# AutoGPTQ/AutoGPTQ

Hardware: AMD Instinct MI355X
Metric: int4 g128 QuantLinear fwd GB/s + tokens/s, Llama-7B shapes (higher is better)
Workload: dtype f16; 1 GPU; Llama-7B linear shapes (4096->4096 x4, 4096->11008 x2, 11008->4096) x 32 blocks = 224 layers, int4 g128 no act-order, M=1 rows per step, 128 launches/step in one hipGraph (q|k|v and gate|up of a block: one gptq_forward_multi launch each); layers=224, launches=128, parallelism=single

## Files before the change

autogptq_amd/csrc/gemv_shared.cuh:

```cuda
#pragma once
#include <type_traits>

#include "common.cuh"
#include "launch.h"

namespace gptq {

struct GemvParams {
    const unsigned* qweight;
    const unsigned* qzeros;
    const void* scales;
    const int* g_idx;
    const int* perm;
    const void* bias;
    const void* x;
    void* out;
    float* partial;
    int M, K, N, group_size, zero_mode;
    int units_total, units_per_split, chunk_units, ksplit;
    int gu_shift;
    int pair_off;
};
hipError_t launch_gemv_generic(const gptq_layer_t& L, const GemvPlan& pl, const GemvParams& p, hipStream_t st);

template <int CTRL> __device__ __forceinline__ float dpp_add(float v) {
    const int r = __builtin_amdgcn_update_dpp(0, __builtin_bit_cast(int, v), CTRL, 0xf, 0xf, false);
    return v + __builtin_bit_cast(float, r);
}
template <int LN> __device__ __forceinline__ float row_slot_sum(float v) {
    if constexpr (LN <= 4) v = dpp_add<0x124>(v);
    if constexpr (LN <= 8) v = dpp_add<0x128>(v);
    if constexpr (LN <= 16) v += __shfl_xor(v, 16, 64);
    if constexpr (LN <= 32) v += __shfl_xor(v, 32, 64);
    return v;
}

__device__ __forceinline__ float kslot_sum_swap(float v) {
    const unsigned u = __builtin_bit_cast(unsigned, v);
    const auto a = __builtin_amdgcn_permlane16_swap(u, u, false, false);
    const unsigned a0 = a[0], a1 = a[1];
    const unsigned s = as_u32(as_f32(a0) + as_f32(a1));
    const auto b = __builtin_amdgcn_permlane32_swap(s, s, false, false);
    const unsigned b0 = b[0], b1 = b[1];
    return as_f32(b0) + as_f32(b1);
}
template <int WN, int STRIDE> __device__ __forceinline__ float tree_sum(const float* r) {
    float a[WN];
#pragma unroll
    for (int w = 0; w < WN; ++w) a[w] = r[w * STRIDE];
#pragma unroll
    for (int off = 1; off < WN; off <<= 1)
#pragma unroll
        for (int i = 0; i < WN; i += 2 * off) a[i] += a[i + off];
    return a[0];
}
template <int WN, int STRIDE> __device__ __forceinline__ float seq_sum(const float* r) {
    float a[WN];
#pragma unroll
    for (int w = 0; w < WN; ++w) a[w] = r[w * STRIDE];
    float t = 0.f;
#pragma unroll
    for (int w = 0; w < WN; ++w) t += a[w];
    return t;
}

template <typename T> struct Mma4;
template <> struct Mma4<f16> {
    typedef _Float16 v4 __attribute__((ext_vector_type(4)));
    static __device__ __forceinline__ f32x4 run(u32x2 a, u32x2 b, f32x4 c) {
        return __builtin_amdgcn_mfma_f32_4x4x4f16(__builtin_bit_cast(v4, a), __builtin_bit_cast(v4, b), c, 0, 0, 0);
    }
    static __device__ __forceinline__ unsigned short bits_of_int(int d) { return as_u16((f16)(short)d); }
};
template <> struct Mma4<bf16> {
    typedef short v4 __attribute__((ext_vector_type(4)));
    static __device__ __forceinline__ f32x4 run(u32x2 a, u32x2 b, f32x4 c) {
        return __builtin_amdgcn_mfma_f32_4x4x4bf16_1k(__builtin_bit_cast(v4, a), __builtin_bit_cast(v4, b), c, 0, 0, 0);
    }
    static __device__ __forceinline__ unsigned short bits_of_int(int d) { return (unsigned short)(as_u32((float)d) >> 16); }
};

__device__ __forceinline__ void dma16_nt(const void* gsrc, unsigned lds_dst) {
    unsigned keep;
    asm volatile("s_mov_b32 %0, m0\n\ts_mov_b32 m0, %2\n\ts_nop 0\n\tglobal_load_lds_dwordx4 %1, off nt\n\ts_mov_b32 m0, %0"
                 : "=&s"(keep) : "v"(gsrc), "s"(lds_dst) : "memory");
}

template <bool NT> __device__ __forceinline__ void dma16_sv(__attribute__((address_space(1))) const char* sbase, unsigned voff, unsigned lds_dst) {
    if constexpr (NT) asm volatile("s_mov_b32 m0, %2\n\ts_nop 0\n\tglobal_load_lds_dwordx4 %0, %1 nt" : : "v"(voff), "s"(sbase), "s"(lds_dst) : "memory");
    else asm volatile("s_mov_b32 m0, %2\n\ts_nop 0\n\tglobal_load_lds_dwordx4 %0, %1" : : "v"(voff), "s"(sbase), "s"(lds_dst) : "memory");
}
template <int ROWS, bool NT>
__device__ __forceinline__ void stage_rows(__attribute__((address_space(1))) const char* const (&base)[ROWS], const unsigned (&lds)[ROWS], int tid, int w64, int step, int pieces) {
    if (w64 >= pieces) return;
    if (tid < pieces) {
#pragma unroll
        for (int r = 0; r < ROWS; ++r) dma16_sv<NT>(base[r], (unsigned)tid * 16u, lds[r] + (unsigned)w64 * 16u);
    }
    if (w64 + step >= pieces) return;
    if (tid + step < pieces) {
#pragma unroll
        for (int r = 0; r < ROWS; ++r) dma16_sv<NT>(base[r], (unsigned)(tid + step) * 16u, lds[r] + (unsigned)(w64 + step) * 16u);
    }
    if (__builtin_expect(w64 + 2 * step >= pieces, 1)) return;
    for (int a = 2 * step; w64 + a < pieces; a += step) {
        if (tid + a < pieces) {
#pragma unroll
            for (int r = 0; r < ROWS; ++r) dma16_sv<NT>(base[r], (unsigned)(tid + a) * 16u, lds[r] + (unsigned)(w64 + a) * 16u);
        }
    }
}
__device__ __forceinline__ int scalar_ge(int a, int b) {
    int r;
    asm("s_cmp_ge_i32 %1, %2\n\ts_cselect_b32 %0, 1, 0" : "=s"(r) : "s"(a), "s"(b) : "scc");
    return r;
}

struct GemvSeg {
    const unsigned* qweight;
    const unsigned* qzeros;
    const void* scales;
    const void* bias;
    void* out;
    int N;
    int blk_end;
    int col0;
    int pad_;
};
struct GemvStreamParams {
    GemvSeg seg[4];
    const void* x;
    unsigned long long* gran;
    unsigned* epochs;
    unsigned* err;
    int nseg, M, K, zero_mode, units_total, units_per_split, ksplit, gu_shift, nsum;
    unsigned max_spins;
};

template <int CT, int MT, typename T, typename PP = GemvStreamParams, typename SG = GemvSeg>
__device__ __forceinline__ void stream_finish(const PP& p, const SG& sg, int strip, int sidx, int ks, int N, const float* red, T* stage = nullptr) {
    const int tid = threadIdx.x, lane = tid & 63, wave = tid >> 6, W = blockDim.x >> 6;
    constexpr int E = MT * CT, ES = E + 4;
    unsigned tag = 0;
    if (p.ksplit > 1) {
        unsigned ep;
        asm volatile("s_load_dword %0, %1, 0x0\n\ts_waitcnt lgkmcnt(0)" : "=s"(ep) : "s"(p.epochs + sidx) : "memory");
        tag = 0x7FE00000u | ((ep + 1u) & 0x1FFFFFu);
    }
    const size_t slab = (size_t)p.M * p.nsum;
    bool gave_up = false;
    auto emit = [&](int e, float t) {
        const int m = e / CT, c = e % CT;
        const int n = strip * CT + c;
        if (n >= N || m >= p.M) return;
        if (p.ksplit > 1) {
            const size_t at = (size_t)m * p.nsum + sg.col0 + n;
            if (ks != 0) {
                const unsigned long long g8 = (unsigned long long)as_u32(t) | ((unsigned long long)tag << 32);
                __hip_atomic_store(p.gran + (size_t)(ks - 1) * slab + at, g8, __ATOMIC_RELAXED, __HIP_MEMORY_SCOPE_AGENT);
                return;
            }
            constexpr int KMAX = 8;
            unsigned long long v[KMAX - 1];
            unsigned pending = (1u << (p.ksplit - 1)) - 1u;
            for (unsigned spins = 0; pending; ++spins) {
#pragma unroll
                for (int k = 0; k < KMAX - 1; ++k)
                    if (pending & (1u << k)) v[k] = __hip_atomic_load(p.gran + (size_t)k * slab + at, __ATOMIC_RELAXED, __HIP_MEMORY_SCOPE_AGENT);
#pragma unroll
                for (int k = 0; k < KMAX - 1; ++k)
                    if ((pending & (1u << k)) && (unsigned)(v[k] >> 32) == tag) pending &= ~(1u << k);
                if (pending && spins > p.max_spins) { gave_up = true; break; }
                if (pending) __builtin_amdgcn_s_sleep(2);
            }
#pragma unroll
            for (int k = 0; k < KMAX - 1; ++k)
                if (k < p.ksplit - 1) t += as_f32((unsigned)(v[k] & 0xffffffffu));
#pragma unroll
            for (int k = 0; k < KMAX - 1; ++k)
                if (k < p.ksplit - 1) __hip_atomic_store(p.gran + (size_t)k * slab + at, 0ull, __ATOMIC_RELAXED, __HIP_MEMORY_SCOPE_AGENT);
        }
        if (sg.bias) t += DType<T>::to_f32(((const T*)sg.bias)[n]);
        const T o = DType<T>::from_f32(t);
        if (sg.out) ((T*)sg.out)[(size_t)m * N + n] = o;
        if (stage) stage[m * CT + c] = o;
    };
    if ((W & (W - 1)) == 0) {
        const int lw = __builtin_ctz((unsigned)W);
        const int w_of_lane = lane & (W - 1), e_of_lane = lane >> lw;
        for (int e0 = 0; e0 < E; e0 += 64) {
            const int e = e0 + wave * (64 >> lw) + e_of_lane;
            float t = (e < E) ? red[w_of_lane * ES + e] : 0.f;
            for (int off = 1; off < W; off <<= 1) t += __shfl_xor(t, off, 64);
            if (w_of_lane == 0 && e < E) emit(e, t);
        }
    } else {
        for (int e = tid; e < E; e += blockDim.x) {
            float t = 0.f;
            for (int w = 0; w < W; ++w) t += red[w * ES + e];
            emit(e, t);
        }
    }
    if (p.ksplit > 1 && ks == 0) {
        if (gave_up) __hip_atomic_store(p.err, 1u, __ATOMIC_RELAXED, __HIP_MEMORY_SCOPE_AGENT);
        __syncthreads();
        if (tid == 0) __hip_atomic_store(p.epochs + sidx, (tag & 0x1FFFFFu), __ATOMIC_RELAXED, __HIP_MEMORY_SCOPE_AGENT);
    }
}

template <int LN, int MT, typename T>
__device__ __forceinline__ void stream_epilogue(f32x4 (&acc)[MT], const GemvStreamParams& p, const GemvSeg& sg, int strip, int sidx, int ks, int N,
                                                float* red) {
    constexpr int CT = LN * 4;
    const int tid = threadIdx.x, lane = tid & 63, wave = tid >> 6, W = blockDim.x >> 6;
#pragma unroll
    for (int m = 0; m < MT; ++m)
#pragma unroll
        for (int c = 0; c < 4; ++c) acc[m][c] = row_slot_sum<LN>(acc[m][c]);
    constexpr int E = MT * CT, ES = E + 4;
    if (lane < LN) {
#pragma unroll
        for (int m = 0; m < MT; ++m) *(f32x4*)(red + wave * ES + m * CT + lane * 4) = acc[m];
    }
    __syncthreads();
    stream_finish<CT, MT, T>(p, sg, strip, sidx, ks, N, red);
}


}
```

autogptq_amd/csrc/gemv_tiled_kernel.cuh:

```cuda
#pragma once
#include <cstddef>

#include "gemv_shared.cuh"

namespace gptq {

struct TiledSeg {
    const void* bias;
    void* out;
    int N, col0;
};
struct PeerEpi {
    char* xbuf[2][GPTQ_PEER_MAX];
    unsigned* flags[GPTQ_PEER_MAX];
    unsigned* state;
    int world, rank;
    unsigned row_bytes, col_off_bytes, owners, pad_;
};
struct TiledParams {
    int blk_end[4];
    const void* x;
    int M, K;
    int chunks, chunks_per_split, ksplit, gu_shift, groups, xstride, waves;
    int pair_strips;
    const unsigned* tq[4];
    const void* cst[4];
    const int* perm[4];
    int xraw_off;
    int nseg, nsum;
    unsigned max_spins;
    TiledSeg seg[4];
    unsigned long long* gran;
    unsigned* epochs;
    unsigned* err;
    PeerEpi peer;
};
static_assert(offsetof(TiledParams, perm) == 128, "the entry batch of the decode-copy kernel is the first two cache lines of its arguments");

template <int BITS> struct TiledFmt;
template <> struct TiledFmt<4> { static constexpr int WPL = 4, KPL = 32, REC = 48, ZB = 1; };
template <> struct TiledFmt<8> { static constexpr int WPL = 4, KPL = 16, REC = 64, ZB = 2; };
template <> struct TiledFmt<3> { static constexpr int WPL = 3, KPL = 32, REC = 48, ZB = 1; };
template <> struct TiledFmt<2> { static constexpr int WPL = 2, KPL = 32, REC = 48, ZB = 1; };

#ifdef GPTQ_TILED_STAMPS
#define TILED_STAMP(i) (st_[i] = __builtin_amdgcn_s_memtime() | vz_)
#define TILED_STAMPS_OUT() stamps_out()
#define TILED_HOT_END() return
#else
#define TILED_HOT_END() __builtin_amdgcn_endpgm()
#define TILED_STAMP(i) ((void)0)
#define TILED_STAMPS_OUT() ((void)0)
#endif

template <int N_> struct WordsOf { typedef unsigned type __attribute__((ext_vector_type(N_))); };

template <int BITS, int MT, int U, typename T, int MAXW, int XM = 0, int ZM2 = 0>
__global__ void __launch_bounds__(MAXW * 64, MAXW == 16 ? 4 : 2) gemv_tiled_kernel(TiledParams p) {
#ifdef GPTQ_TILED_STAMPS
    unsigned long long st_[9] = {};
    unsigned vz_;
    asm volatile("v_mov_b32 %0, 0" : "=v"(vz_));
    st_[7] = __builtin_amdgcn_s_memrealtime() | vz_;
    TILED_STAMP(0);
    auto stamps_out = [&]() {
        st_[8] = __builtin_amdgcn_s_memrealtime() | vz_;
        unsigned long long* const dbg = p.gran;
        const int b = (int)blockIdx.x, nb = (int)gridDim.x;
        const int slot = b == 0 ? 0 : (b == 1 ? 1 : (b == nb / 2 ? 2 : (b == nb - 1 ? 3 : -1)));
        if (dbg != nullptr && p.ksplit == 1 && slot >= 0 && (threadIdx.x & 63) == 0) {
#pragma unroll
            for (int i = 0; i < 9; ++i) dbg[(slot * 16 + (int)(threadIdx.x >> 6)) * 16 + i] = st_[i];
        }
    };
#endif
    constexpr bool BF = std::is_same_v<T, bf16>;
    constexpr bool ACT = XM == 1, PEER = XM == 3;
    constexpr bool PAIR = XM == 4;
    constexpr bool MULTI = XM == 5 || XM == 6;
    constexpr int NSTR = PAIR ? 2 : (XM == 5 ? 4 : (XM == 6 ? 2 : 1));
    using F = TiledFmt<BITS>;
    constexpr int WPL = F::WPL, KPL = F::KPL, CKE = 4 * KPL, CHB = 64 * WPL * 4, REC = F::REC, NX = KPL / 8;
    constexpr int LKPL = KPL == 32 ? 5 : 4;
    typedef typename WordsOf<WPL>::type qvec;
    unsigned m_lo, m_hi, m_b, magic;
    asm("s_mov_b32 %0, 0x000f000f" : "=s"(m_lo));
    asm("s_mov_b32 %0, 0x00f000f0" : "=s"(m_hi));
    asm("s_mov_b32 %0, 0x00ff00ff" : "=s"(m_b));
    asm("v_mov_b32 %0, 0x64006400" : "=v"(magic));
    unsigned m2a, m2b, m2c, m2d, m2e;
    asm("s_mov_b32 %0, 0x00030003" : "=s"(m2a));
    asm("s_mov_b32 %0, 0x000c000c" : "=s"(m2b));
    asm("s_mov_b32 %0, 0x00300030" : "=s"(m2c));
    asm("s_mov_b32 %0, 0x00c000c0" : "=s"(m2d));
    asm("s_mov_b32 %0, 0x03000300" : "=s"(m2e));
    unsigned m3a, m3b, m3c;
    asm("s_mov_b32 %0, 0x00070007" : "=s"(m3a));
    asm("s_mov_b32 %0, 0x00380038" : "=s"(m3b));
    asm("s_mov_b32 %0, 0x01c001c0" : "=s"(m3c));
    extern __shared__ __attribute__((aligned(16))) char smem[];
    const int tid = threadIdx.x, lane = tid & 63;
    const int wave = __builtin_amdgcn_readfirstlane(tid >> 6);
    const int col = lane & 15, kb = lane >> 4;
    typedef unsigned u32x16 __attribute__((ext_vector_type(16)));
    typedef unsigned long long u64x8 __attribute__((ext_vector_type(8)));
    typedef unsigned long long u64x4 __attribute__((ext_vector_type(4)));
    static_assert(offsetof(TiledParams, x) == 16 && offsetof(TiledParams, M) == 24 && offsetof(TiledParams, chunks) == 32 && offsetof(TiledParams, pair_strips) == 60 &&
                  offsetof(TiledParams, tq) == 64 && offsetof(TiledParams, cst) == 96 && offsetof(TiledParams, perm) == 128 && offsetof(TiledParams, xraw_off) == 160, "the entry batch");
    u32x16 ha;
    u64x8 hb;
    [[maybe_unused]] u64x4 hp = {};
    [[maybe_unused]] int xraw_off = 0;
    {
        const auto kargs = __builtin_amdgcn_kernarg_segment_ptr();
        if constexpr (ACT)
            asm volatile("s_load_dwordx16 %0, %4, 0x0\n\ts_load_dwordx16 %1, %4, 0x40\n\ts_load_dwordx8 %2, %4, 0x80\n\ts_load_dword %3, %4, 0xa0\n\ts_waitcnt lgkmcnt(0)"
                         : "=&s"(ha), "=&s"(hb), "=&s"(hp), "=&s"(xraw_off) : "s"(kargs));
        else
            asm volatile("s_load_dwordx16 %0, %2, 0x0\n\ts_load_dwordx16 %1, %2, 0x40\n\ts_waitcnt lgkmcnt(0)" : "=&s"(ha), "=&s"(hb) : "s"(kargs));
    }
    const int be0 = (int)ha[0], be1 = (int)ha[1], be2 = (int)ha[2], Mrows = (int)ha[6], K = (int)ha[7], nchunks = (int)ha[8], cps = (int)ha[9], ksplit = (int)ha[10],
              gshift = (int)ha[11], G = (int)ha[12], xstride = (int)ha[13], W = (int)ha[14];
    [[maybe_unused]] const int hstrips = (int)ha[15];
    typedef __attribute__((address_space(1))) const char gchar;
    gchar* const xg = (gchar*)(((unsigned long long)ha[5] << 32) | ha[4]);
    int sidx = blockIdx.x, ks = 0, cb = 0, ce = nchunks, kbeg = 0, kend = K;
    if (__builtin_expect(ksplit != 1, 0)) {
        sidx = (int)blockIdx.x / ksplit; ks = (int)blockIdx.x - sidx * ksplit;
        cb = ks * cps; ce = min(cb + cps, nchunks);
        kbeg = cb * CKE; kend = min(ce * CKE, K);
    }
    unsigned long long tqs_ = hb[0], csts_ = hb[4];
    [[maybe_unused]] unsigned long long perm_ = hp[0];
    int sbase = 0, s = 0;
    if constexpr (ACT)
        asm("s_cmp_ge_i32 %[i], %[e0]\n\ts_cbranch_scc0 1f\n\t"
            "s_mov_b64 %[tq], %[tq1]\n\ts_mov_b64 %[cs], %[cs1]\n\ts_mov_b64 %[pm], %[pm1]\n\ts_mov_b32 %[sb], %[e0]\n\ts_mov_b32 %[s], 1\n\t"
            "s_cmp_ge_i32 %[i], %[e1]\n\ts_cselect_b64 %[tq], %[tq2], %[tq]\n\ts_cselect_b64 %[cs], %[cs2], %[cs]\n\ts_cselect_b64 %[pm], %[pm2], %[pm]\n\ts_cselect_b32 %[sb], %[e1], %[sb]\n\ts_cselect_b32 %[s], 2, %[s]\n\t"
            "s_cmp_ge_i32 %[i], %[e2]\n\ts_cselect_b64 %[tq], %[tq3], %[tq]\n\ts_cselect_b64 %[cs], %[cs3], %[cs]\n\ts_cselect_b64 %[pm], %[pm3], %[pm]\n\ts_cselect_b32 %[sb], %[e2], %[sb]\n\ts_cselect_b32 %[s], 3, %[s]\n"
            "1:"
            : [tq] "+&s"(tqs_), [cs] "+&s"(csts_), [pm] "+&s"(perm_), [sb] "+&s"(sbase), [s] "+&s"(s)
            : [i] "s"(sidx), [e0] "s"(be0), [e1] "s"(be1), [e2] "s"(be2), [tq1] "s"(hb[1]), [tq2] "s"(hb[2]), [tq3] "s"(hb[3]), [cs1] "s"(hb[5]), [cs2] "s"(hb[6]), [cs3] "s"(hb[7]),
              [pm1] "s"(hp[1]), [pm2] "s"(hp[2]), [pm3] "s"(hp[3])
            : "scc");
    else
        asm("s_cmp_ge_i32 %[i], %[e0]\n\ts_cbranch_scc0 1f\n\t"
            "s_mov_b64 %[tq], %[tq1]\n\ts_mov_b64 %[cs], %[cs1]\n\ts_mov_b32 %[sb], %[e0]\n\ts_mov_b32 %[s], 1\n\t"
            "s_cmp_ge_i32 %[i], %[e1]\n\ts_cselect_b64 %[tq], %[tq2], %[tq]\n\ts_cselect_b64 %[cs], %[cs2], %[cs]\n\ts_cselect_b32 %[sb], %[e1], %[sb]\n\ts_cselect_b32 %[s], 2, %[s]\n\t"
            "s_cmp_ge_i32 %[i], %[e2]\n\ts_cselect_b64 %[tq], %[tq3], %[tq]\n\ts_cselect_b64 %[cs], %[cs3], %[cs]\n\ts_cselect_b32 %[sb], %[e2], %[sb]\n\ts_cselect_b32 %[s], 3, %[s]\n"
            "1:"
            : [tq] "+&s"(tqs_), [cs] "+&s"(csts_), [sb] "+&s"(sbase), [s] "+&s"(s)
            : [i] "s"(sidx), [e0] "s"(be0), [e1] "s"(be1), [e2] "s"(be2), [tq1] "s"(hb[1]), [tq2] "s"(hb[2]), [tq3] "s"(hb[3]), [cs1] "s"(hb[5]), [cs2] "s"(hb[6]), [cs3] "s"(hb[7])
            : "scc");
    gchar* const tqs = (gchar*)tqs_;
    gchar* const csts = (gchar*)csts_;
    [[maybe_unused]] const int* const permp = (const int*)perm_;
    const int strip = sidx - sbase;
    const int Wh = NSTR == 4 ? (W >> 2) : (NSTR == 2 ? (W >> 1) : W);
    const int sel = NSTR == 1 ? 0 : (scalar_ge(wave, Wh) + (NSTR == 4 ? scalar_ge(wave, 2 * Wh) + scalar_ge(wave, 3 * Wh) : 0));
    const int wv = NSTR == 1 ? wave : wave - sel * Wh;
    const int strip_w = PAIR ? strip + sel * hstrips : (MULTI ? strip * NSTR + sel : strip);
    char* const xs = smem;
    char* const cs = smem + (size_t)MT * xstride;
    const unsigned crec = (unsigned)G * (unsigned)REC;
    const size_t cpad = ((size_t)crec + 15) & ~(size_t)15;
    float* const red = (float*)(cs + NSTR * cpad);
    gchar* const tb = tqs + (size_t)(unsigned)strip_w * ((unsigned)nchunks * (unsigned)CHB);
    gchar* const cg = csts + (size_t)(unsigned)(MULTI ? strip * NSTR : strip) * crec;
    const unsigned t_lane = (unsigned)lane * (WPL * 4u);
    auto stage_all = [&]() __attribute__((always_inline)) {
        const unsigned xs_lds = (unsigned)(size_t)(__attribute__((address_space(3))) char*)xs, cs_lds = (unsigned)(size_t)(__attribute__((address_space(3))) char*)cs;
        const int w64 = wave * 64, step = W * 64;
        gchar* xrow[MT];
        unsigned xdst[MT];
        if constexpr (XM == 0 || XM == 3 || XM == 4 || MULTI) {
#pragma unroll
            for (int m = 0; m < MT; ++m) {
                xrow[m] = xg + (unsigned)((m == 0 ? 0 : min(m, Mrows - 1)) * K + kbeg) * 2u;
                xdst[m] = xs_lds + m * xstride;
            }
            stage_rows<MT, false>(xrow, xdst, tid, w64, step, (kend - kbeg) >> 3);
        } else if constexpr (ACT) {
#pragma unroll
            for (int m = 0; m < MT; ++m) {
                xrow[m] = xg + (unsigned)((m == 0 ? 0 : min(m, Mrows - 1)) * K) * 2u;
                xdst[m] = xs_lds + (unsigned)xraw_off + m * (K * 2 + 16);
            }
            stage_rows<MT, false>(xrow, xdst, tid, w64, step, K >> 3);
        }
        const int cpieces = (int)(crec >> 4) * (MULTI ? NSTR : 1);
        if constexpr (PAIR) {
            gchar* const crow[2] = {cg, cg + (size_t)(unsigned)hstrips * crec};
            const unsigned cdst[2] = {cs_lds, cs_lds + (unsigned)cpad};
            stage_rows<2, true>(crow, cdst, tid, w64, step, cpieces);
        } else {
            gchar* const crow[1] = {cg};
            const unsigned cdst[1] = {cs_lds};
            stage_rows<1, true>(crow, cdst, tid, w64, step, cpieces);
        }
    };
#ifndef GPTQ_TILED_WEIGHTS_FIRST
    stage_all();
#endif
    typedef int i32x4 __attribute__((ext_vector_type(4)));
    i32x4 pa[2][2] = {};
    const int apieces = ACT ? (kend - kbeg) >> 3 : 0;
    if constexpr (ACT) {
        const int* const pg = permp + kbeg;
        if (tid < apieces) { pa[0][0] = *(const i32x4*)(pg + tid * 8); pa[0][1] = *(const i32x4*)(pg + tid * 8 + 4); }
        if (tid + W * 64 < apieces) { pa[1][0] = *(const i32x4*)(pg + (tid + W * 64) * 8); pa[1][1] = *(const i32x4*)(pg + (tid + W * 64) * 8 + 4); }
    }
    auto x_gather = [&]() {
        const int* const pg = permp + kbeg;
        const char* const xraw = smem + xraw_off;
        for (int pc0 = tid; pc0 < apieces; pc0 += 2 * W * 64) {
            const int pcb = pc0 + W * 64;
            const bool two = pcb < apieces;
            if (pc0 != tid) {
                pa[0][0] = *(const i32x4*)(pg + pc0 * 8); pa[0][1] = *(const i32x4*)(pg + pc0 * 8 + 4);
                if (two) { pa[1][0] = *(const i32x4*)(pg + pcb * 8); pa[1][1] = *(const i32x4*)(pg + pcb * 8 + 4); }
            }
#pragma unroll
            for (int m = 0; m < MT; ++m) {
                const unsigned short* xr = (const unsigned short*)(xraw + (size_t)m * (K * 2 + 16));
#pragma unroll
                for (int h = 0; h < 2; ++h) {
                    if (h == 1 && !two) break;
                    unsigned short v[8];
#pragma unroll
                    for (int i = 0; i < 8; ++i) v[i] = xr[pa[h][i >> 2][i & 3]];
                    u32x4 o;
#pragma unroll
                    for (int i = 0; i < 4; ++i) o[i] = (unsigned)v[2 * i] | ((unsigned)v[2 * i + 1] << 16);
                    *(u32x4*)(xs + (size_t)m * xstride + (size_t)(h ? pcb : pc0) * 16) = o;
                }
            }
        }
    };
#if defined(GPTQ_TILED_ZM)
    constexpr bool ZM = BITS == 4 && MT <= 4 && (GPTQ_TILED_ZM == 2 || (GPTQ_TILED_ZM == 1 && BF));
#else
    constexpr bool ZM = BITS == 4 && BF && (MT == 4 || (MT == 2 && ZM2 == 1));
#endif
#ifdef GPTQ_TILED_NO_XS
    constexpr bool XS = false;
#else
    constexpr bool XS = BF && BITS == 4 && MT <= 2 && !ZM;
#endif
    constexpr bool XC = BF && MT <= 2 && !XS && !ZM;
    using MM = std::conditional_t<XC, f16, T>;
    constexpr int ES = MT * 16 + 4;
    float* const xe = red + W * ES;
    auto x_to_f16 = [&]() {
        const int prow = (kend - kbeg) >> 3, total = prow * MT;
        for (int i0 = 0; i0 < total; i0 += W * 64) {
            const int idx = i0 + tid;
            const bool ok = idx < total;
            int m = 0, pc = ok ? idx : 0;
            if constexpr (MT > 1) { m = pc / prow; pc -= m * prow; }
            u32x4* const at = (u32x4*)(xs + (size_t)m * xstride + (size_t)pc * 16);
            u32x4 v = {0u, 0u, 0u, 0u};
            if (ok) v = *at;
            unsigned mx = 0u;
#pragma unroll
            for (int i = 0; i < 4; ++i) {
                const unsigned a = v[i] & 0x7fff7fffu;
                mx = max(mx, max(a & 0xffffu, a >> 16));
            }
            mx = max(mx, (unsigned)__shfl_xor((int)mx, 1, 64));
            if constexpr (NX == 4) mx = max(mx, (unsigned)__shfl_xor((int)mx, 2, 64));
            const int E = (int)((mx >> 7) & 0xffu);
            const int ms = min(max(268 - E, 1), 253);
            const float mult = __builtin_bit_cast(float, (unsigned)ms << 23);
#pragma unroll
            for (int i = 0; i < 4; ++i) {
                const float lo = __builtin_bit_cast(float, v[i] << 16) * mult, hi = __builtin_bit_cast(float, v[i] & 0xffff0000u) * mult;
                v[i] = __builtin_bit_cast(unsigned, __builtin_amdgcn_cvt_pkrtz(lo, hi));
            }
            if (ok) {
                *at = v;
                if ((pc & (NX - 1)) == 0) xe[(pc / NX) * 4 + m] = __builtin_bit_cast(float, (unsigned)(254 - ms) << 23);
            }
        }
        __syncthreads();
    };
    auto x_sums = [&]() {
        const int prow = (kend - kbeg) >> 3, total = prow * MT;
        for (int i0 = 0; i0 < total; i0 += W * 64) {
            const int idx = i0 + tid;
            const bool ok = idx < total;
            int m = 0, pc = ok ? idx : 0;
            if constexpr (MT > 1) { m = pc / prow; pc -= m * prow; }
            u32x4 v = {0u, 0u, 0u, 0u};
            if (ok) v = *(const u32x4*)(xs + (size_t)m * xstride + (size_t)pc * 16);
            float sm = 0.f;
#pragma unroll
            for (int i = 0; i < 4; ++i) sm += __builtin_bit_cast(float, v[i] << 16) + __builtin_bit_cast(float, v[i] & 0xffff0000u);
            sm += __shfl_xor(sm, 1, 64);
            if constexpr (NX == 4) sm += __shfl_xor(sm, 2, 64);
            if (ok && (pc & (NX - 1)) == 0) xe[(pc / NX) * 4 + m] = sm;
        }
        __syncthreads();
    };
    const char* const xl = xs + (size_t)min(lane & 3, MT - 1) * xstride + kb * (KPL * 2);
    const char* const xl2 = xs + (size_t)min(4 + (lane & 3), MT - 1) * xstride + kb * (KPL * 2);
    float acc[MT];
#pragma unroll
    for (int m = 0; m < MT; ++m) acc[m] = 0.f;
    const f16x2 k960 = {(f16)960.f, (f16)960.f}, k896 = {(f16)896.f, (f16)896.f}, k1008 = {(f16)1008.f, (f16)1008.f};
    const f16x2 r16 = {(f16)0.0625f, (f16)0.0625f}, r8 = {(f16)0.125f, (f16)0.125f}, r64 = {(f16)0.015625f, (f16)0.015625f};
    const f16x2 k768 = {(f16)768.f, (f16)768.f}, k1020 = {(f16)1020.f, (f16)1020.f}, r4 = {(f16)0.25f, (f16)0.25f}, r256 = {(f16)0.00390625f, (f16)0.00390625f};
    auto bits_of = [&](f16x2 hv) -> unsigned {
        if constexpr (BF && !XC) {
            const bf16x2 o = {(bf16)(float)hv[0], (bf16)(float)hv[1]};
            return __builtin_bit_cast(unsigned, o);
        } else {
            return __builtin_bit_cast(unsigned, hv);
        }
    };
    constexpr int E = MT * 16, NE = (MULTI ? NSTR : 1) * E;
    const int n_t = (MULTI ? strip * NSTR + tid / E : strip) * 16 + (tid & 15);
    float bv0 = 0.f, bv1 = 0.f;
    typedef __attribute__((address_space(1))) T gT;
    int N = 0;
    const void* biasp = nullptr;
    void* outp = nullptr;
    auto seg_request = [&]() __attribute__((always_inline)) {
        int sl = s;
        asm volatile("" : "+s"(sl) : : "memory");
        N = p.seg[sl].N; biasp = p.seg[sl].bias; outp = p.seg[sl].out;
    };
    auto seg_pin = [&]() __attribute__((always_inline)) { asm volatile("" : "+s"(N), "+s"(biasp), "+s"(outp)); };
    bool staged = false;
    for (int cbase = cb; cbase < ce; cbase += Wh * U) {
        const int c0 = cbase + wv * U;
        qvec q[U];
#pragma unroll
        for (int j = 0; j < U; ++j) q[j] = __builtin_nontemporal_load((const __attribute__((address_space(1))) qvec*)(tb + ((unsigned)min(c0 + j, ce - 1) * (unsigned)CHB + t_lane)));
        if (!staged) {
            TILED_STAMP(1);
            seg_request();
#ifdef GPTQ_TILED_WEIGHTS_FIRST
            stage_all();
            asm volatile("s_waitcnt vmcnt(0)" ::: "memory");
#else
            asm volatile("s_waitcnt vmcnt(%0)" ::"n"(U) : "memory");
#endif
            if constexpr (ACT) {
                __syncthreads();
                x_gather();
            }
            __syncthreads();
            if constexpr (XC) x_to_f16();
            if constexpr (XS) x_sums();
            seg_pin();
            if (biasp != nullptr && tid < NE && n_t < (PAIR ? N >> 1 : N)) {
                bv0 = DType<T>::to_f32(((const gT*)biasp)[n_t]);
                if constexpr (PAIR) bv1 = DType<T>::to_f32(((const gT*)biasp)[n_t + (N >> 1)]);
            }
            TILED_STAMP(2);
            staged = true;
        }
#ifdef GPTQ_TILED_STAMPS
        if (cbase + Wh * U >= ce) { asm volatile("s_waitcnt vmcnt(0)" ::: "memory"); TILED_STAMP(3); }
#endif
#pragma unroll
        for (int j = 0; j < U; ++j) {
            const int cc = min(c0 + j, ce - 1);
            const int k0 = cc * CKE + kb * KPL;
            const bool live = (c0 + j < ce) && (k0 < K);
            const int g = min(k0 >> LKPL >> gshift, G - 1);
            const char* cp = cs + (NSTR > 1 ? (size_t)sel * cpad : (size_t)0) + g * REC;
            const unsigned short sraw = *(const unsigned short*)(cp + col * 2);
            unsigned z;
            if constexpr (F::ZB == 1) z = *(const unsigned char*)(cp + 32 + col);
            else z = *(const unsigned short*)(cp + 32 + col * 2);
            u32x4 xa[NX];
#pragma unroll
            for (int w = 0; w < NX; ++w) xa[w] = *(const u32x4*)(xl + ((unsigned)(cc - cb) * (unsigned)(CKE * 2) + w * 16u));
            u32x4 xb[MT > 4 ? NX : 1];
            if constexpr (MT > 4) {
#pragma unroll
                for (int w = 0; w < NX; ++w) xb[w] = *(const u32x4*)(xl2 + ((unsigned)(cc - cb) * (unsigned)(CKE * 2) + w * 16u));
            }
            const f16x2 c1 = as_f16x2(z * 0x00010001u + 0xE400E400u);
            const qvec qv = q[j];
            f32x4 accg = {0.f, 0.f, 0.f, 0.f}, accg2 = {0.f, 0.f, 0.f, 0.f};
            auto mm = [&](int pc, int hf, unsigned b0, unsigned b1) __attribute__((always_inline)) {
                accg = Mma4<MM>::run(u32x2{xa[pc][hf * 2], xa[pc][hf * 2 + 1]}, u32x2{b0, b1}, accg);
                if constexpr (MT > 4) accg2 = Mma4<MM>::run(u32x2{xb[pc][hf * 2], xb[pc][hf * 2 + 1]}, u32x2{b0, b1}, accg2);
            };
            if constexpr (BITS == 4 && ZM) {
                unsigned mgz;
                asm("v_mov_b32 %0, %1" : "=v"(mgz) : "n"(BF ? 0x43004300 : 0x64006400));
                const unsigned nz = z * 0x00010001u + (BF ? 0xC300C300u : 0xE400E400u);
                f32x4 accz = {0.f, 0.f, 0.f, 0.f};
#pragma unroll
                for (int w = 0; w < 4; ++w) {
                    const unsigned qw = qv[w];
                    mm(w, 0, (qw & m_lo) | mgz, ((qw >> 4) & m_lo) | mgz);
                    mm(w, 1, ((qw >> 8) & m_lo) | mgz, ((qw >> 12) & m_lo) | mgz);
                    accz = Mma4<MM>::run(u32x2{xa[w][0], xa[w][1]}, u32x2{nz, nz}, accz);
                    accz = Mma4<MM>::run(u32x2{xa[w][2], xa[w][3]}, u32x2{nz, nz}, accz);
                }
                accg += accz;
            } else if constexpr (BITS == 4 && XS) {
                unsigned magicb;
                asm("v_mov_b32 %0, 0x43004300" : "=v"(magicb));
#pragma unroll
                for (int w = 0; w < 4; ++w) {
                    const unsigned qw = qv[w];
                    mm(w, 0, (qw & m_lo) | magicb, ((qw >> 4) & m_lo) | magicb);
                    mm(w, 1, ((qw >> 8) & m_lo) | magicb, ((qw >> 12) & m_lo) | magicb);
                }
            } else if constexpr (BITS == 4) {
                const f16x2 c2 = c1 + k960;
#pragma unroll
                for (int w = 0; w < 4; ++w) {
                    const unsigned qw = qv[w], q8 = qw >> 8;
                    const f16x2 h0 = as_f16x2((qw & m_lo) | magic) + c1;
                    const f16x2 h1 = as_f16x2((qw & m_hi) | magic) * r16 + c2;
                    const f16x2 h2 = as_f16x2((q8 & m_lo) | magic) + c1;
                    const f16x2 h3 = as_f16x2((q8 & m_hi) | magic) * r16 + c2;
                    mm(w, 0, bits_of(h0), bits_of(h1));
                    mm(w, 1, bits_of(h2), bits_of(h3));
                }
            } else if constexpr (BITS == 2) {
                const f16x2 c4 = c1 + k768, c16 = c1 + k960, c64 = c1 + k1008, c256 = c1 + k1020;
#pragma unroll
                for (int w = 0; w < 2; ++w) {
                    const unsigned t = qv[w], t10 = t >> 10;
                    const unsigned p0 = bits_of(as_f16x2((t & m2a) | magic) + c1);
                    const unsigned p1 = bits_of(as_f16x2((t & m2b) | magic) * r4 + c4);
                    const unsigned p2 = bits_of(as_f16x2((t & m2c) | magic) * r16 + c16);
                    const unsigned p3 = bits_of(as_f16x2((t & m2d) | magic) * r64 + c64);
                    const unsigned p4 = bits_of(as_f16x2((t & m2e) | magic) * r256 + c256);
                    const unsigned p5 = bits_of(as_f16x2((t10 & m2a) | magic) + c1);
                    const unsigned p6 = bits_of(as_f16x2((t10 & m2b) | magic) * r4 + c4);
                    const unsigned p7 = bits_of(as_f16x2((t10 & m2c) | magic) * r16 + c16);
                    mm(2 * w, 0, p0, p1);
                    mm(2 * w, 1, p2, p3);
                    mm(2 * w + 1, 0, p4, p5);
                    mm(2 * w + 1, 1, p6, p7);
                }
            } else if constexpr (BITS == 8) {
#pragma unroll
                for (int w = 0; w < 4; ++w) {
                    const unsigned qw = qv[w], q8 = qw >> 8;
                    const f16x2 h0 = as_f16x2((qw & m_b) | magic) + c1;
                    const f16x2 h1 = as_f16x2((q8 & m_b) | magic) + c1;
                    mm(w >> 1, w & 1, bits_of(h0), bits_of(h1));
                }
            } else {
                const f16x2 c3 = c1 + k896;
                const f16x2 c6 = c1 + k1008;
                unsigned pr[16];
#pragma unroll
                for (int w = 0; w < 3; ++w) {
                    const unsigned t = qv[w], t6 = t >> 6;
                    pr[5 * w + 0] = bits_of(as_f16x2((t & m3a) | magic) + c1);
                    pr[5 * w + 1] = bits_of(as_f16x2((t & m3b) | magic) * r8 + c3);
                    pr[5 * w + 2] = bits_of(as_f16x2((t & m3c) | magic) * r64 + c6);
                    pr[5 * w + 3] = bits_of(as_f16x2((t6 & m3b) | magic) * r8 + c3);
                    pr[5 * w + 4] = bits_of(as_f16x2((t6 & m3c) | magic) * r64 + c6);
                }
                const unsigned e = ((qv[0] >> 15) & 0x00010001u) | ((qv[1] >> 14) & 0x00020002u) | ((qv[2] >> 13) & 0x00040004u);
                pr[15] = bits_of(as_f16x2(e | magic) + c1);
#pragma unroll
                for (int i = 0; i < 8; ++i) mm(i >> 1, i & 1, pr[2 * i], pr[2 * i + 1]);
            }
            const float sc = DType<T>::to_f32(__builtin_bit_cast(T, sraw));
            if constexpr (XS) {
                const float* const xv = xe + ((cc - cb) * 4 + kb) * 4;
                const float zc = (float)(128u + z);
#pragma unroll
                for (int m = 0; m < MT; ++m) acc[m] = live ? fmaf(sc, fmaf(-zc, xv[m], accg[m]), acc[m]) : acc[m];
            } else if constexpr (XC) {
                const float* const xi = xe + ((cc - cb) * 4 + kb) * 4;
#pragma unroll
                for (int m = 0; m < MT; ++m) acc[m] = live ? fmaf(sc * xi[m], accg[m], acc[m]) : acc[m];
            } else {
#pragma unroll
                for (int m = 0; m < MT; ++m) acc[m] = live ? fmaf(sc, m < 4 ? accg[m] : accg2[m - 4], acc[m]) : acc[m];
            }
        }
    }
    TILED_STAMP(4);
#pragma unroll
    for (int m = 0; m < MT; ++m) acc[m] = kslot_sum_swap(acc[m]);
    if (__builtin_expect(!staged, 0)) {
        seg_request();
        seg_pin();
        __syncthreads();
    }
    gT* const outg = (gT*)outp;
    if (lane < 16) {
#pragma unroll
        for (int m = 0; m < MT; ++m) red[wave * ES + m * 16 + lane] = acc[m];
    }
    __syncthreads();
    TILED_STAMP(5);
    if constexpr (PAIR) {
        const int NH = N >> 1;
        if (tid < E) {
            const int m = tid >> 4;
            const float* const r = red + tid;
            float s0 = 0.f, s1 = 0.f;
            if (Wh == 4) { s0 = seq_sum<4, ES>(r); s1 = seq_sum<4, ES>(r + 4 * ES); }
            else if (MAXW == 16 && Wh == 8) { s0 = seq_sum<8, ES>(r); s1 = seq_sum<8, ES>(r + 8 * ES); }
            else if (Wh == 2) { s0 = seq_sum<2, ES>(r); s1 = seq_sum<2, ES>(r + 2 * ES); }
            else for (int w = 0; w < Wh; ++w) { s0 += r[w * ES]; s1 += r[(Wh + w) * ES]; }
            if (m < Mrows && n_t < NH) {
                if (biasp != nullptr) { s0 += bv0; s1 += bv1; }
                const float g = s0 / (1.f + __expf(-s0));
                outg[(size_t)m * NH + n_t] = DType<T>::from_f32(g * s1);
            }
        }
        TILED_STAMP(6);
        TILED_STAMPS_OUT();
        return;
    }
    if constexpr (MULTI) {
        const bool lean = (NE <= W * 64) & ((((MAXW == 16 ? 0x114u : 0x14u) >> (Wh & 31)) & 1u) != 0u);
        if (__builtin_expect(lean, 1)) {
            if (tid < NE) {
                const int s4 = tid / E, r = tid & (E - 1), m = r >> 4;
                float t;
                constexpr int WHOT = (XM == 6 && MT <= 2) ? 2 : 4;
                if (__builtin_expect(Wh == WHOT, 1)) t = seq_sum<WHOT, ES>(red + s4 * WHOT * ES + r);
                else if (Wh == 6 - WHOT) t = seq_sum<6 - WHOT, ES>(red + s4 * (6 - WHOT) * ES + r);
                else if constexpr (MAXW == 16) t = seq_sum<8, ES>(red + s4 * 8 * ES + r);
                else t = 0.f;
                if (m < Mrows && n_t < N) {
                    if (biasp != nullptr) t += bv0;
                    outg[(size_t)m * N + n_t] = DType<T>::from_f32(t);
                }
            }
            TILED_STAMP(6);
            TILED_STAMPS_OUT();
            TILED_HOT_END();
        }
        for (int e = tid; e < NSTR * MT * 16; e += W * 64) {
            const int s4 = e / (MT * 16), r = e - s4 * (MT * 16), m = r >> 4, c = r & 15, n = (strip * NSTR + s4) * 16 + c;
            float t = 0.f;
            for (int w = 0; w < Wh; ++w) t += red[(s4 * Wh + w) * ES + r];
            if (m < Mrows && n < N) {
                if (biasp) t += DType<T>::to_f32(((const T*)biasp)[n]);
                ((T*)outp)[(size_t)m * N + n] = DType<T>::from_f32(t);
            }
        }
        return;
    }
    if constexpr (!PEER) {
        const bool lean = (ksplit == 1) & ((((MAXW == 16 ? 0x10110u : 0x110u) >> (W & 31)) & 1u) != 0u);
        if (__builtin_expect(lean, 1)) {
            if (tid < E) {
                const int m = tid >> 4;
                const float* const r = red + tid;
                float t;
                constexpr int WHOT = MAXW == 16 ? 16 : 4;
                if (__builtin_expect(W == WHOT, 1)) t = tree_sum<WHOT, ES>(r);
                else if (MAXW == 8 || W == 8) t = tree_sum<8, ES>(r);
                else t = tree_sum<4, ES>(r);
                if (m < Mrows && n_t < N) {
                    if (biasp != nullptr) t += bv0;
                    outg[(size_t)m * N + n_t] = DType<T>::from_f32(t);
                }
            }
            TILED_STAMP(6);
            TILED_STAMPS_OUT();
            TILED_HOT_END();
        }
    }
    T* const stage = PEER ? (T*)xs : nullptr;
    const TiledSeg sg{biasp, outp, N, ksplit != 1 ? p.seg[s].col0 : 0};
    stream_finish<16, MT, T, TiledParams, TiledSeg>(p, sg, strip, sidx, ks, N, red, stage);
    if constexpr (PEER) if (ks == 0) {
        const int pworld = p.peer.world;
        __syncthreads();
        const unsigned e = __hip_atomic_load(p.peer.state, __ATOMIC_RELAXED, __HIP_MEMORY_SCOPE_AGENT) + 1u;
        if (tid < pworld * MT * 2) {
            const int r = tid / (MT * 2), m = (tid >> 1) % MT, q = tid & 1;
            if (m < Mrows) {
                const u32x4 v = *(const u32x4*)((const char*)stage + m * 32 + q * 16);
                char* const dst = p.peer.xbuf[e & 1u][r] + (size_t)m * p.peer.row_bytes + p.peer.col_off_bytes + (size_t)strip * 32 + q * 16;
                asm volatile("global_store_dwordx4 %0, %1, off sc0 sc1\n\ts_nop 1" ::"v"(dst), "v"(v) : "memory");
            }
        }
    }
}

template <int U, int XM> constexpr int tiled_maxw() { return (U == 2 || XM == 5) ? 16 : 8; }
int tiled_max_waves(int u, int nstr);
template <int BITS, int MT, int U, typename T, int XM>
static hipError_t launch_tiled_one(const TiledPlan& pl, const TiledParams& p, hipStream_t st) {
    constexpr int MAXW = tiled_maxw<U, XM>();
    if (pl.waves > MAXW) return hipErrorInvalidValue;
    if constexpr (BITS == 4 && MT == 2 && std::is_same_v<T, bf16> && (XM == 0 || XM == 1)) {
        if (pl.zm2) {
            hipLaunchKernelGGL((gemv_tiled_kernel<BITS, MT, U, T, MAXW, XM, 1>), dim3(pl.strips_total * pl.ksplit), dim3(pl.waves * 64), pl.lds_bytes, st, p);
            return hipGetLastError();
        }
    }
    hipLaunchKernelGGL((gemv_tiled_kernel<BITS, MT, U, T, MAXW, XM>), dim3(pl.strips_total * pl.ksplit), dim3(pl.waves * 64), pl.lds_bytes, st, p);
    return hipGetLastError();
}
template <int BITS, int MT, typename T, int XM>
static hipError_t launch_tiled_u(const TiledPlan& pl, const TiledParams& p, hipStream_t st) {
    switch (pl.u) {
        case 2: if constexpr (!(XM == 6 && MT <= 2)) return launch_tiled_one<BITS, MT, 2, T, XM>(pl, p, st); else return hipErrorInvalidValue;
        case 4: return launch_tiled_one<BITS, MT, 4, T, XM>(pl, p, st);
        default: return hipErrorInvalidValue;
    }
}
template <int BITS, typename T, int XM>
static hipError_t launch_tiled_mt(const TiledPlan& pl, const TiledParams& p, hipStream_t st) {
    constexpr bool LOW_OK = XM != 5 && (XM != 6 || BITS == 4);
    if constexpr (!LOW_OK) {
        if (pl.mt != 4 && pl.mt != 8) return hipErrorInvalidValue;
    }
    switch (pl.mt) {
        case 1: if constexpr (LOW_OK) return launch_tiled_u<BITS, 1, T, XM>(pl, p, st); else return hipErrorInvalidValue;
        case 2: if constexpr (LOW_OK) return launch_tiled_u<BITS, 2, T, XM>(pl, p, st); else return hipErrorInvalidValue;
        case 4: return launch_tiled_u<BITS, 4, T, XM>(pl, p, st);
        case 8: if constexpr (XM != 3 && XM != 4 && BITS != 2) return launch_tiled_u<BITS, 8, T, XM>(pl, p, st); else return hipErrorInvalidValue;
        default: return hipErrorInvalidValue;
    }
}
template <typename T, int XM>
static hipError_t launch_tiled_bits(const TiledPlan& pl, const TiledParams& p, hipStream_t st) {
    switch (pl.bits) {
        case 4: return launch_tiled_mt<4, T, XM>(pl, p, st);
        case 8: return launch_tiled_mt<8, T, XM>(pl, p, st);
        case 3: return launch_tiled_mt<3, T, XM>(pl, p, st);
        case 2:
            if constexpr (XM == 0 || XM == 1) { if (pl.mt <= 4) return launch_tiled_mt<2, T, XM>(pl, p, st); }
            return hipErrorInvalidValue;
        default: return hipErrorInvalidValue;
    }
}

template <int XM>
static hipError_t grant_tiled_lds() {
    hipError_t e = hipSuccess;
    auto grant = [&](auto kern) { hipError_t r = hipFuncSetAttribute((const void*)kern, hipFuncAttributeMaxDynamicSharedMemorySize, 160 * 1024); if (e == hipSuccess) e = r; };
    auto grant_mt = [&](auto mt) {
        constexpr int MT = decltype(mt)::value;
        auto grant_u = [&](auto bu, auto uu) {
            constexpr int B = decltype(bu)::value, U = decltype(uu)::value;
            constexpr int MAXW = tiled_maxw<U, XM>();
            grant(gemv_tiled_kernel<B, MT, U, f16, MAXW, XM>); grant(gemv_tiled_kernel<B, MT, U, bf16, MAXW, XM>);
            if constexpr (B == 4 && MT == 2 && (XM == 0 || XM == 1)) grant(gemv_tiled_kernel<B, MT, U, bf16, MAXW, XM, 1>);
        };
        using I2 = std::integral_constant<int, 2>; using I3 = std::integral_constant<int, 3>; using I4 = std::integral_constant<int, 4>; using I8 = std::integral_constant<int, 8>;
        grant_u(I4{}, I2{}); grant_u(I4{}, I4{});
        grant_u(I8{}, I2{}); grant_u(I8{}, I4{}); grant_u(I3{}, I2{}); grant_u(I3{}, I4{});
        if constexpr ((XM == 0 || XM == 1) && MT <= 4) { grant_u(I2{}, I2{}); grant_u(I2{}, I4{}); }
    };
    if constexpr (XM != 5 && XM != 6) { grant_mt(std::integral_constant<int, 1>{}); grant_mt(std::integral_constant<int, 2>{}); }
    if constexpr (XM == 6) {
        grant(gemv_tiled_kernel<4, 1, 4, f16, 8, 6>); grant(gemv_tiled_kernel<4, 1, 4, bf16, 8, 6>);
        grant(gemv_tiled_kernel<4, 2, 4, f16, 8, 6>); grant(gemv_tiled_kernel<4, 2, 4, bf16, 8, 6>);
    }
    grant_mt(std::integral_constant<int, 4>{});
    if constexpr (XM != 3 && XM != 4) grant_mt(std::integral_constant<int, 8>{});
    return e;
}

}
```

Before: 3587 GB/s.

## Stage x and scale slices per wave to drop the block-wide staging barrier

Adds a private staging mode in which each wave DMAs only the x pieces and scale/zero records its own chunks need, using exec-masked global_load_lds. The next round's slice is prefetched while the last weight word is still in flight. This removes the cooperative stage_all plus __syncthreads before compute, so waves start as soon as their own data lands rather than waiting on the slowest wave. In exchange the loop is split into two rounds, more small DMAs are issued, and scale records may be loaded redundantly by several waves. The mode is disabled for act-order, multi-strip and the bf16 conversion paths.

```diff
diff --git a/autogptq_amd/csrc/gemv_shared.cuh b/autogptq_amd/csrc/gemv_shared.cuh
--- a/autogptq_amd/csrc/gemv_shared.cuh
+++ b/autogptq_amd/csrc/gemv_shared.cuh
@@ -89,6 +89,11 @@
 template <bool NT> __device__ __forceinline__ void dma16_sv(__attribute__((address_space(1))) const char* sbase, unsigned voff, unsigned lds_dst) {
     if constexpr (NT) asm volatile("s_mov_b32 m0, %2\n\ts_nop 0\n\tglobal_load_lds_dwordx4 %0, %1 nt" : : "v"(voff), "s"(sbase), "s"(lds_dst) : "memory");
     else asm volatile("s_mov_b32 m0, %2\n\ts_nop 0\n\tglobal_load_lds_dwordx4 %0, %1" : : "v"(voff), "s"(sbase), "s"(lds_dst) : "memory");
+}
+template <bool NT> __device__ __forceinline__ void dma16_svm(__attribute__((address_space(1))) const char* sbase, unsigned voff, unsigned lds_dst, unsigned long long mask) {
+    unsigned long long keep;
+    if constexpr (NT) asm volatile("s_and_saveexec_b64 %0, %4\n\ts_mov_b32 m0, %3\n\ts_nop 0\n\tglobal_load_lds_dwordx4 %1, %2 nt\n\ts_mov_b64 exec, %0" : "=&s"(keep) : "v"(voff), "s"(sbase), "s"(lds_dst), "s"(mask) : "memory", "scc");
+    else asm volatile("s_and_saveexec_b64 %0, %4\n\ts_mov_b32 m0, %3\n\ts_nop 0\n\tglobal_load_lds_dwordx4 %1, %2\n\ts_mov_b64 exec, %0" : "=&s"(keep) : "v"(voff), "s"(sbase), "s"(lds_dst), "s"(mask) : "memory", "scc");
 }
 template <int ROWS, bool NT>
 __device__ __forceinline__ void stage_rows(__attribute__((address_space(1))) const char* const (&base)[ROWS], const unsigned (&lds)[ROWS], int tid, int w64, int step, int pieces) {
diff --git a/autogptq_amd/csrc/gemv_tiled_kernel.cuh b/autogptq_amd/csrc/gemv_tiled_kernel.cuh
--- a/autogptq_amd/csrc/gemv_tiled_kernel.cuh
+++ b/autogptq_amd/csrc/gemv_tiled_kernel.cuh
@@ -58,7 +58,7 @@
 template <int BITS, int MT, int U, typename T, int MAXW, int XM = 0, int ZM2 = 0>
 __global__ void __launch_bounds__(MAXW * 64, MAXW == 16 ? 4 : 2) gemv_tiled_kernel(TiledParams p) {
 #ifdef GPTQ_TILED_STAMPS
-    unsigned long long st_[9] = {};
+    unsigned long long st_[10] = {};
     unsigned vz_;
     asm volatile("v_mov_b32 %0, 0" : "=v"(vz_));
     st_[7] = __builtin_amdgcn_s_memrealtime() | vz_;
@@ -70,7 +70,7 @@
         const int slot = b == 0 ? 0 : (b == 1 ? 1 : (b == nb / 2 ? 2 : (b == nb - 1 ? 3 : -1)));
         if (dbg != nullptr && p.ksplit == 1 && slot >= 0 && (threadIdx.x & 63) == 0) {
 #pragma unroll
-            for (int i = 0; i < 9; ++i) dbg[(slot * 16 + (int)(threadIdx.x >> 6)) * 16 + i] = st_[i];
+            for (int i = 0; i < 10; ++i) dbg[(slot * 16 + (int)(threadIdx.x >> 6)) * 16 + i] = st_[i];
         }
     };
 #endif
@@ -199,8 +199,34 @@
             stage_rows<1, true>(crow, cdst, tid, w64, step, cpieces);
         }
     };
+#ifndef GPTQ_TILED_PRIVATE
+#define GPTQ_TILED_PRIVATE 2
+#endif
+#if defined(GPTQ_TILED_WEIGHTS_FIRST)
+    constexpr bool PRIV = false;
+#else
+    constexpr bool PRIV = NSTR == 1 && !ACT && !(BF && MT <= 2 && !(BITS == 4 && MT == 2 && ZM2 == 1)) && (((GPTQ_TILED_PRIVATE) >> (U == 2 ? 0 : 1)) & 1) != 0;
+#endif
+    [[maybe_unused]] gchar* xrow_w[MT];
+    if constexpr (PRIV) {
+#pragma unroll
+        for (int m = 0; m < MT; ++m) xrow_w[m] = xg + (unsigned)((m == 0 ? 0 : min(m, Mrows - 1)) * K + kbeg) * 2u;
+    }
+    auto stage_own = [&](int c0) __attribute__((always_inline)) {
+        const unsigned xs_lds = (unsigned)(size_t)(__attribute__((address_space(3))) char*)xs, cs_lds = (unsigned)(size_t)(__attribute__((address_space(3))) char*)cs;
+        constexpr int PPC = CKE / 8;
+        const int cl = min(c0 + U, ce);
+        const int p0 = (c0 - cb) * PPC;
+        const int np = min((cl - cb) * PPC, (kend - kbeg) >> 3) - p0;
+        const unsigned long long xmask = __builtin_amdgcn_ballot_w64(lane < np);
+#pragma unroll
+        for (int m = 0; m < MT; ++m) dma16_svm<false>(xrow_w[m], (unsigned)(p0 + lane) * 16u, xs_lds + (unsigned)(m * xstride + p0 * 16), xmask);
+        const int g0 = min((c0 * 4) >> gshift, G - 1), g1 = min((cl * 4 - 1) >> gshift, G - 1);
+        const int nc = c0 < ce ? ((g1 - g0 + 1) * REC) >> 4 : 0;
+        dma16_svm<true>(cg, (unsigned)(g0 * REC + lane * 16), cs_lds + (unsigned)(g0 * REC), __builtin_amdgcn_ballot_w64(lane < nc));
+    };
 #ifndef GPTQ_TILED_WEIGHTS_FIRST
-    stage_all();
+    if constexpr (!PRIV) stage_all();
 #endif
     typedef int i32x4 __attribute__((ext_vector_type(4)));
     i32x4 pa[2][2] = {};
@@ -248,6 +274,7 @@
     constexpr bool XS = BF && BITS == 4 && MT <= 2 && !ZM;
 #endif
     constexpr bool XC = BF && MT <= 2 && !XS && !ZM;
+    static_assert(!PRIV || (!XC && !XS), "the passes over the staged x (x_to_f16, x_sums) read what other waves staged: cooperative staging and its barrier");
     using MM = std::conditional_t<XC, f16, T>;
     constexpr int ES = MT * 16 + 4;
     float* const xe = red + W * ES;
@@ -332,12 +359,19 @@
     };
     auto seg_pin = [&]() __attribute__((always_inline)) { asm volatile("" : "+s"(N), "+s"(biasp), "+s"(outp)); };
     bool staged = false;
-    for (int cbase = cb; cbase < ce; cbase += Wh * U) {
+    constexpr int ROUNDS = PRIV ? 2 : 1;
+#pragma unroll
+    for (int rnd = 0; rnd < ROUNDS; ++rnd)
+    for (int cbase = rnd == 0 ? cb : cb + Wh * U; cbase < ce; cbase = PRIV && rnd == 0 ? ce : cbase + Wh * U) {
+        const bool first = PRIV ? rnd == 0 : !staged;
         const int c0 = cbase + wv * U;
+        if constexpr (PRIV) {
+            if (first && c0 < ce) stage_own(c0);
+        }
         qvec q[U];
 #pragma unroll
         for (int j = 0; j < U; ++j) q[j] = __builtin_nontemporal_load((const __attribute__((address_space(1))) qvec*)(tb + ((unsigned)min(c0 + j, ce - 1) * (unsigned)CHB + t_lane)));
-        if (!staged) {
+        if (first) {
             TILED_STAMP(1);
             seg_request();
 #ifdef GPTQ_TILED_WEIGHTS_FIRST
@@ -350,7 +384,7 @@
                 __syncthreads();
                 x_gather();
             }
-            __syncthreads();
+            if constexpr (!PRIV) __syncthreads();
             if constexpr (XC) x_to_f16();
             if constexpr (XS) x_sums();
             seg_pin();
@@ -359,13 +393,24 @@
                 if constexpr (PAIR) bv1 = DType<T>::to_f32(((const gT*)biasp)[n_t + (N >> 1)]);
             }
             TILED_STAMP(2);
+#ifdef GPTQ_TILED_STAMPS
+            asm volatile("s_waitcnt vmcnt(0)" ::: "memory");
+            TILED_STAMP(9);
+#endif
             staged = true;
+        } else if constexpr (PRIV) {
+            asm volatile("s_waitcnt vmcnt(%0)" ::"n"(U) : "memory");
         }
 #ifdef GPTQ_TILED_STAMPS
         if (cbase + Wh * U >= ce) { asm volatile("s_waitcnt vmcnt(0)" ::: "memory"); TILED_STAMP(3); }
 #endif
 #pragma unroll
         for (int j = 0; j < U; ++j) {
+            if constexpr (PRIV) if (j == U - 1) {
+                asm volatile("" : "+v"(q[U - 1]));
+                stage_own(c0 + Wh * U);
+                asm volatile("" : "+v"(q[U - 1]));
+            }
             const int cc = min(c0 + j, ce - 1);
             const int k0 = cc * CKE + kb * KPL;
             const bool live = (c0 + j < ce) && (k0 < K);
```

Result: no change. 3582 GB/s (-0.1%).
